# WangXuan95/NBLIC-Image-Compression

Hardware: AMD Instinct MI355X
Metric: Mpixel/s encode (bit-exact) 4096x4096 gray -e1 lossless (higher is better)
Workload: dtype u8

## Files before the change

include/nblic_amd.h:

```cpp
#ifndef NBLIC_AMD_H
#define NBLIC_AMD_H

#include <stddef.h>
#include <stdint.h>

#ifdef __cplusplus
extern "C" {
#endif

#define NBLIC_MAX_HEIGHT     65535
#define NBLIC_MAX_WIDTH      65535
#define NBLIC_MAX_IMG_SIZE   100000000
#define QNBLIC_MAX_HEIGHT    65535
#define QNBLIC_MAX_WIDTH     65535
#define QNBLIC_MAX_IMG_SIZE  100000000


int NBLICcompress(int verbose, unsigned char *p_buf, unsigned char *p_img, int height, int width,
                  int *p_near, int *p_effort);

int NBLICdecompress(int verbose, unsigned char *p_buf, unsigned char *p_img, int *p_height, int *p_width,
                    int *p_near, int *p_effort);

int QNBLICcompress(uint16_t *p_buf, unsigned char *p_img, int height, int width);
// ... 5 lines not shown

nblic_amd_ctx *nblic_amd_create(int device, int n_slots, int n_coders);

nblic_amd_ctx *nblic_amd_create_ex(int device, int n_groups, int group_size, int n_coders, int n_host_buffers);
void nblic_amd_destroy(nblic_amd_ctx *ctx);

int nblic_amd_encode_batch(nblic_amd_ctx *ctx, int n_images, const unsigned char *const *imgs, int imgs_on_device,
                           const int *heights, const int *widths, unsigned char *const *outs,
                           const size_t *out_caps, long *out_lens);

typedef struct nblic_amd_batch nblic_amd_batch;
nblic_amd_batch *nblic_amd_encode_batch_begin(nblic_amd_ctx *ctx, int n_images, const unsigned char *const *imgs,
                                              int imgs_on_device, const int *heights, const int *widths,
                                              unsigned char *const *outs, const size_t *out_caps, long *out_lens);
int nblic_amd_encode_batch_end(nblic_amd_ctx *ctx, nblic_amd_batch *batch);

int nblic_amd_qencode_batch(nblic_amd_ctx *ctx, int n_images, const unsigned char *const *imgs, int imgs_on_device,
                            const int *heights, const int *widths, uint16_t *const *outs, const size_t *out_caps_words,
                            long *out_len_words);

int nblic_amd_encode_batch_modes(nblic_amd_ctx *ctx, int n_images, const unsigned char *const *imgs, int imgs_on_device,
                                 const int *heights, const int *widths, const int *nears, const int *efforts,
                                 unsigned char *const *outs, const size_t *out_caps, long *out_lens,
                                 unsigned char *const *recons);

int nblic_amd_decode_batch(nblic_amd_ctx *ctx, int n_images, const unsigned char *const *streams, const size_t *stream_lens,
                           unsigned char *const *imgs, const size_t *img_caps, int *heights, int *widths, int *nears,
                           int *efforts, int *status);

int nblic_amd_set_device_coder(nblic_amd_ctx *ctx, int n_packs, int min_outstanding);
void nblic_amd_device_coder_stats(nblic_amd_ctx *ctx, double *bins, long *packs, long *images);

int nblic_amd_copy_stats(nblic_amd_ctx *ctx, long out[4]);

void nblic_amd_set_max_pixels(nblic_amd_ctx *ctx, long max_pixels);

void nblic_amd_set_serial_rows(nblic_amd_ctx *ctx, int rows);
long nblic_amd_serial_launches(nblic_amd_ctx *ctx);

void nblic_amd_set_long_chains(nblic_amd_ctx *ctx, int min_records, int block_records);
int nblic_amd_long_chain_stats(nblic_amd_ctx *ctx, long counts[8], int reset);

int nblic_amd_lsq_redo_counts(nblic_amd_ctx *ctx, unsigned long long counts[2], int reset);

int nblic_amd_serial_plan(int decode, int effort, int images, int width, int whole_streams);

typedef struct nblic_amd_stream nblic_amd_stream;
nblic_amd_stream *nblic_amd_stream_begin(nblic_amd_ctx *ctx, const unsigned char *img, int img_on_device, int height, int width,
                                         int near, int effort, int band_rows);
nblic_amd_stream *nblic_amd_stream_resume(nblic_amd_ctx *ctx, const unsigned char *img, int img_on_device, const void *checkpoint,
                                          size_t checkpoint_bytes);
int nblic_amd_stream_run(nblic_amd_stream *s, double budget_seconds, unsigned char *out, size_t out_cap, size_t *out_len);
size_t nblic_amd_stream_checkpoint(nblic_amd_stream *s, void *buf, size_t cap);
int nblic_amd_stream_check(nblic_amd_ctx *ctx, const void *checkpoint, size_t bytes);
int nblic_amd_stream_progress(nblic_amd_stream *s, int *rows_done, unsigned long long *bytes_total, unsigned char sha256[32], double *model_ms);
int nblic_amd_stream_recon(nblic_amd_stream *s, unsigned char *plane, int *first_row, int *end_row);
void nblic_amd_stream_end(nblic_amd_stream *s);
int nblic_amd_stream_set_index(nblic_amd_stream *s, int every_rows);
size_t nblic_amd_stream_index(nblic_amd_stream *s, void *buf, size_t cap);
int nblic_amd_stream_set_front(nblic_amd_stream *s, int front);

typedef struct nblic_amd_dstream nblic_amd_dstream;
nblic_amd_dstream *nblic_amd_dstream_begin(nblic_amd_ctx *ctx, int band_rows);
nblic_amd_dstream *nblic_amd_dstream_resume(nblic_amd_ctx *ctx, const void *checkpoint, size_t bytes);
int nblic_amd_dstream_check(nblic_amd_ctx *ctx, const void *checkpoint, size_t bytes);
int nblic_amd_dstream_feed(nblic_amd_dstream *d, const unsigned char *bytes, size_t n, int final_);
// ... 375 lines not shown
```

nblic-image-compression_amd/__init__.py:

```python
from __future__ import annotations

import ctypes as C
import os
import subprocess
import weakref
from typing import List, Optional, Sequence, Tuple

import numpy as np


_HERE = os.path.dirname(os.path.abspath(__file__))
LIB_PATH = os.environ.get("NBLIC_AMD_LIB") or os.path.join(_HERE, "libnblic_amd.so")
CSRC = os.path.join(_HERE, "csrc")
INCLUDE = os.path.join(os.path.dirname(_HERE), "include", "nblic_amd.h")

_u8p = C.POINTER(C.c_uint8)
_lib = None

EXPORTS = (
    "NBLICcompress", "NBLICdecompress", "QNBLICcompress", "QNBLICdecompress", "QNBLICcompressMultiThread",
    "nblic_amd_create", "nblic_amd_create_ex", "nblic_amd_destroy", "nblic_amd_encode_batch", "nblic_amd_encode_batch_begin", "nblic_amd_encode_batch_end", "nblic_amd_qencode_batch", "nblic_amd_set_max_pixels",
    "nblic_amd_enable_timing", "nblic_amd_stage_times", "nblic_amd_last_launches", "nblic_amd_last_stats", "nblic_amd_debug_stage", "nblic_amd_debug_live", "nblic_amd_debug_takes", "nblic_amd_debug_pack_rows", "nblic_amd_debug_device_code", "nblic_amd_debug_model_stages", "nblic_amd_debug_back_half", "nblic_amd_debug_entropy_front",
    "nblic_amd_encode_batch_modes", "nblic_amd_decode_batch", "nblic_amd_serial_selftest",
    "nblic_amd_set_serial_rows", "nblic_amd_serial_launches", "nblic_amd_set_long_chains", "nblic_amd_long_chain_stats", "nblic_amd_lsq_redo_counts", "nblic_amd_serial_plan", "nblic_amd_lsq_probe", "nblic_amd_set_feed_chunk", "nblic_amd_last_fed_bytes",
    "nblic_amd_stream_begin", "nblic_amd_stream_resume", "nblic_amd_stream_run", "nblic_amd_stream_checkpoint", "nblic_amd_stream_progress",
    "nblic_amd_stream_recon", "nblic_amd_stream_end", "nblic_amd_stream_check",
    "nblic_amd_dstream_begin", "nblic_amd_dstream_resume", "nblic_amd_dstream_check", "nblic_amd_dstream_feed", "nblic_amd_dstream_info",
    "nblic_amd_dstream_run", "nblic_amd_dstream_progress", "nblic_amd_dstream_checkpoint", "nblic_amd_dstream_end",
    "nblic_amd_index_check", "nblic_amd_index_build", "nblic_amd_decode_indexed", "nblic_amd_decode_rows",
    "nblic_amd_stream_set_index", "nblic_amd_stream_index", "nblic_amd_set_index_round", "nblic_amd_stream_set_front",
    "nblic_amd_encode_batch_indexed", "nblic_amd_index_bytes", "nblic_amd_indexed_batch_split",
    "nblic_amd_qencode_batch_indexed", "nblic_amd_debug_q_entropy",
    "nblic_amd_set_device_qcoder", "nblic_amd_device_qcoder_stats", "nblic_amd_qcoder_selftest", "nblic_amd_debug_q_rans_host", "nblic_amd_debug_device_q_entropy",
    "nblic_amd_decode_batch_indexed", "nblic_amd_indexed_decode_split", "nblic_amd_indexed_decode_plan", "nblic_amd_debug_index_kernels",
    "nblic_amd_index_build_batch", "nblic_amd_index_build_split", "nblic_amd_index_build_plan", "nblic_amd_debug_index_capture",
    "nblic_amd_index_pack", "nblic_amd_index_pack_bound", "nblic_amd_index_unpack", "nblic_amd_index_unpacked_bytes", "nblic_amd_index_is_packed", "nblic_amd_debug_index_unpack",
    "nblic_amd_decode_batch_indexed_to", "nblic_amd_decode_batch_to", "nblic_amd_debug_deliver_host", "nblic_amd_debug_deliver",
    "nblic_amd_decode_batch_indexed_to_ex", "nblic_amd_decode_batch_to_ex", "nblic_amd_deliver_stats", "nblic_amd_debug_deliver_host_ex", "nblic_amd_debug_deliver_ex",
    "nblic_amd_encode_batch_modes_from_to",
    "nblic_amd_encode_batch_modes_from", "nblic_amd_qencode_batch_from", "nblic_amd_encode_batch_indexed_from", "nblic_amd_qencode_batch_indexed_from",
    "nblic_amd_collect_stats", "nblic_amd_collect_ms", "nblic_amd_debug_collect_host", "nblic_amd_debug_collect",
    "nblic_amd_debug_collect_ref_host", "nblic_amd_debug_collect_ref", "nblic_amd_debug_deliver_ref_host", "nblic_amd_debug_deliver_ref",
    "nblic_amd_color_plan", "nblic_amd_color_choose", "nblic_amd_color_mode_valid", "nblic_amd_color_mode_ref", "nblic_amd_color_plan_stats",
    "nblic_amd_encode_batch_modes_from_color", "nblic_amd_qencode_batch_from_color", "nblic_amd_encode_batch_indexed_from_color",
    "nblic_amd_qencode_batch_indexed_from_color", "nblic_amd_decode_batch_to_ex_color", "nblic_amd_decode_batch_indexed_to_ex_color",
    "nblic_amd_debug_color_cost_host", "nblic_amd_debug_color_cost",
    "nblic_amd_stack_plan", "nblic_amd_stack_choose", "nblic_amd_stack_slice_mode", "nblic_amd_stack_mode_valid", "nblic_amd_stack_modes_valid", "nblic_amd_stack_plan_stats",
    "nblic_amd_encode_batch_modes_from_stack", "nblic_amd_qencode_batch_from_stack", "nblic_amd_encode_batch_indexed_from_stack",
    "nblic_amd_qencode_batch_indexed_from_stack", "nblic_amd_decode_batch_to_ex_stack", "nblic_amd_decode_batch_indexed_to_ex_stack",
    "nblic_amd_debug_stack_deliver_host", "nblic_amd_debug_stack_deliver", "nblic_amd_debug_stack_cost_host", "nblic_amd_debug_stack_cost",
    "nblic_amd_deep_plan", "nblic_amd_deep_choose", "nblic_amd_deep_mode_valid", "nblic_amd_deep_plan_stats",
    "nblic_amd_encode_batch_modes_from_deep", "nblic_amd_qencode_batch_from_deep", "nblic_amd_encode_batch_indexed_from_deep",
    "nblic_amd_qencode_batch_indexed_from_deep", "nblic_amd_decode_batch_to_ex_deep", "nblic_amd_decode_batch_indexed_to_ex_deep",
    "nblic_amd_debug_deep_collect_host", "nblic_amd_debug_deep_collect", "nblic_amd_debug_deep_deliver_host", "nblic_amd_debug_deep_deliver",
    "nblic_amd_debug_deep_cost_host", "nblic_amd_debug_deep_cost",
    "nblic_amd_cli_main", "nblic_amd_cli_parse", "nblic_amd_read_gray", "nblic_amd_write_gray",
    "nblic_amd_set_device_coder", "nblic_amd_device_coder_stats", "nblic_amd_copy_stats",
    "nblic_amd_range_code", "nblic_amd_range_code_multi", "nblic_amd_range_code_chunked", "nblic_amd_range_code_packs", "nblic_amd_pack_groups_host", "nblic_amd_selftest", "nblic_amd_syn1", "nblic_amd_version",
)


def build(force: bool = False) -> str:
    srcs = [os.path.join(CSRC, f) for f in os.listdir(CSRC)] + [INCLUDE]
    stale = force or not os.path.exists(LIB_PATH) or any(os.path.getmtime(s) > os.path.getmtime(LIB_PATH) for s in srcs)
    if stale:
        r = subprocess.run(["make", "-C", CSRC], capture_output=True, text=True)
        if r.returncode != 0:
            raise RuntimeError("building libnblic_amd.so failed:\n" + r.stdout + r.stderr)
    return LIB_PATH


def load_library() -> C.CDLL:
    global _lib
    if _lib is not None:
        return _lib
    if not os.path.exists(LIB_PATH):
        raise RuntimeError(f"{LIB_PATH} is missing: run __graft_entry__.build() (hipcc, gfx950). "
                           "There is no CPU fallback for the NBLIC hot path.")
    lib = C.CDLL(LIB_PATH)
    ip = C.POINTER(C.c_int)
    lib.NBLICcompress.restype = C.c_int
    lib.NBLICcompress.argtypes = [C.c_int, _u8p, _u8p, C.c_int, C.c_int, ip, ip]
    lib.NBLICdecompress.restype = C.c_int
    lib.NBLICdecompress.argtypes = [C.c_int, _u8p, _u8p, ip, ip, ip, ip]
    u16p = C.POINTER(C.c_uint16)
    lib.QNBLICcompress.restype = C.c_int
    lib.QNBLICcompress.argtypes = [u16p, _u8p, C.c_int, C.c_int]
    lib.QNBLICcompressMultiThread.restype = C.c_int
    lib.QNBLICcompressMultiThread.argtypes = [u16p, _u8p, C.c_int, C.c_int]
    lib.QNBLICdecompress.restype = C.c_int
# ... 19 lines not shown
    lib.nblic_amd_encode_batch_modes.argtypes = [C.c_void_p, C.c_int, C.POINTER(C.c_void_p), C.c_int, ip, ip, ip, ip,
                                                 C.POINTER(C.c_void_p), C.POINTER(C.c_size_t), C.POINTER(C.c_long), C.POINTER(C.c_void_p)]
    lib.nblic_amd_decode_batch.restype = C.c_int
    lib.nblic_amd_decode_batch.argtypes = [C.c_void_p, C.c_int, C.POINTER(C.c_void_p), C.POINTER(C.c_size_t), C.POINTER(C.c_void_p),
                                           C.POINTER(C.c_size_t), ip, ip, ip, ip, ip]
    lib.nblic_amd_serial_selftest.restype = C.c_int
    lib.nblic_amd_serial_selftest.argtypes = [C.c_void_p]
    lib.nblic_amd_cli_main.restype = C.c_int
    lib.nblic_amd_cli_main.argtypes = [C.c_int, C.POINTER(C.c_char_p)]
    lib.nblic_amd_cli_parse.restype = None
    lib.nblic_amd_cli_parse.argtypes = [C.c_int, C.POINTER(C.c_char_p), ip, C.c_char_p, C.c_char_p, C.c_size_t]
    lib.nblic_amd_read_gray.restype = C.c_int
    lib.nblic_amd_read_gray.argtypes = [C.c_char_p, _u8p, C.c_size_t, ip, ip]
    lib.nblic_amd_write_gray.restype = C.c_int
    lib.nblic_amd_write_gray.argtypes = [C.c_char_p, _u8p, C.c_int, C.c_int, C.c_int]
    lib.nblic_amd_set_device_coder.restype = C.c_int
    lib.nblic_amd_set_device_coder.argtypes = [C.c_void_p, C.c_int, C.c_int]
    lib.nblic_amd_device_coder_stats.restype = None
    lib.nblic_amd_device_coder_stats.argtypes = [C.c_void_p, C.POINTER(C.c_double), C.POINTER(C.c_long), C.POINTER(C.c_long)]
    lib.nblic_amd_set_max_pixels.restype = None
    lib.nblic_amd_set_max_pixels.argtypes = [C.c_void_p, C.c_long]
    lib.nblic_amd_set_serial_rows.restype = None
    lib.nblic_amd_set_serial_rows.argtypes = [C.c_void_p, C.c_int]
    lib.nblic_amd_serial_launches.restype = C.c_long
    lib.nblic_amd_serial_launches.argtypes = [C.c_void_p]
    if hasattr(lib, "nblic_amd_set_long_chains"):
        lib.nblic_amd_set_long_chains.restype = None
        lib.nblic_amd_set_long_chains.argtypes = [C.c_void_p, C.c_int, C.c_int]
        lib.nblic_amd_long_chain_stats.restype = C.c_int
        lib.nblic_amd_long_chain_stats.argtypes = [C.c_void_p, C.POINTER(C.c_long), C.c_int]
    if hasattr(lib, "nblic_amd_copy_stats"):
        lib.nblic_amd_copy_stats.restype = C.c_int
        lib.nblic_amd_copy_stats.argtypes = [C.c_void_p, C.POINTER(C.c_long)]
    lib.nblic_amd_lsq_redo_counts.restype = C.c_int
    lib.nblic_amd_lsq_redo_counts.argtypes = [C.c_void_p, C.POINTER(C.c_ulonglong), C.c_int]
    lib.nblic_amd_serial_plan.restype = C.c_int
    lib.nblic_amd_serial_plan.argtypes = [C.c_int, C.c_int, C.c_int, C.c_int, C.c_int]
    lib.nblic_amd_lsq_probe.restype = C.c_int
    lib.nblic_amd_lsq_probe.argtypes = [C.c_void_p, C.c_int, C.c_int, C.c_int, C.POINTER(C.c_double), C.POINTER(C.c_int8), ip,
                                        C.POINTER(C.c_double), C.POINTER(C.c_longlong)]
    lib.nblic_amd_set_feed_chunk.restype = None
    lib.nblic_amd_set_feed_chunk.argtypes = [C.c_void_p, C.c_size_t]
    lib.nblic_amd_last_fed_bytes.restype = C.c_long
    lib.nblic_amd_last_fed_bytes.argtypes = [C.c_void_p]
    lib.nblic_amd_stream_begin.restype = C.c_void_p
    lib.nblic_amd_stream_begin.argtypes = [C.c_void_p, C.c_void_p, C.c_int, C.c_int, C.c_int, C.c_int, C.c_int, C.c_int]
    lib.nblic_amd_stream_resume.restype = C.c_void_p
    lib.nblic_amd_stream_resume.argtypes = [C.c_void_p, C.c_void_p, C.c_int, C.c_void_p, C.c_size_t]
    lib.nblic_amd_stream_run.restype = C.c_int
    lib.nblic_amd_stream_run.argtypes = [C.c_void_p, C.c_double, C.c_void_p, C.c_size_t, C.POINTER(C.c_size_t)]
    lib.nblic_amd_stream_checkpoint.restype = C.c_size_t
    lib.nblic_amd_stream_checkpoint.argtypes = [C.c_void_p, C.c_void_p, C.c_size_t]
    lib.nblic_amd_stream_progress.restype = C.c_int
    lib.nblic_amd_stream_progress.argtypes = [C.c_void_p, ip, C.POINTER(C.c_ulonglong), C.c_void_p, C.POINTER(C.c_double)]
    lib.nblic_amd_stream_recon.restype = C.c_int
    lib.nblic_amd_stream_recon.argtypes = [C.c_void_p, C.c_void_p, ip, ip]
    lib.nblic_amd_stream_end.restype = None
    lib.nblic_amd_stream_end.argtypes = [C.c_void_p]
    lib.nblic_amd_stream_check.restype = C.c_int
    lib.nblic_amd_stream_check.argtypes = [C.c_void_p, C.c_void_p, C.c_size_t]
    lib.nblic_amd_dstream_begin.restype = C.c_void_p
    lib.nblic_amd_dstream_begin.argtypes = [C.c_void_p, C.c_int]
    lib.nblic_amd_dstream_resume.restype = C.c_void_p
    lib.nblic_amd_dstream_resume.argtypes = [C.c_void_p, C.c_void_p, C.c_size_t]
    lib.nblic_amd_dstream_check.restype = C.c_int
    lib.nblic_amd_dstream_check.argtypes = [C.c_void_p, C.c_void_p, C.c_size_t]
# ... 2374 lines not shown
            raise RuntimeError("nblic_amd_debug_index_unpack failed (%d)" % rc)
        res = []
        for out, stride, (_, _, walk, first_out) in zip(outs, strides, tasks):
            used = (int(walk) - int(first_out)) * int(stride)
            res.append((out[:used].reshape(-1, int(stride)), out[used:used + 256]))
        return res

    def set_index_round(self, segments: int):
        self.lib.nblic_amd_set_index_round(self.handle, int(segments))

    def set_serial_rows(self, rows: int):
        self.lib.nblic_amd_set_serial_rows(self.handle, rows)

    def serial_launches(self) -> int:
        return int(self.lib.nblic_amd_serial_launches(self.handle))

    LONG_CHAIN_COUNTS = ("s2_met", "s2_table", "s2_serial", "s3_split", "s3_accepted", "s3_missed")

    def set_long_chains(self, min_records: int = 0, block_records: int = 0):
        self.lib.nblic_amd_set_long_chains(self.handle, min_records, block_records)

    def long_chain_stats(self, reset: bool = False) -> dict:
        v = (C.c_long * 8)()
        if self.lib.nblic_amd_long_chain_stats(self.handle, v, int(reset)) != 0:
            raise RuntimeError("nblic_amd_long_chain_stats failed")
        return dict(zip(self.LONG_CHAIN_COUNTS, (int(x) for x in v)))

    def copy_stats(self) -> dict:
        v = (C.c_long * 4)()
        if self.lib.nblic_amd_copy_stats(self.handle, v) != 0:
            raise RuntimeError("nblic_amd_copy_stats failed")
        return {"engine": int(v[0]), "runtime": int(v[1]), "fallbacks": int(v[2]), "available": bool(v[3])}

    def lsq_redo_counts(self, reset: bool = False) -> Tuple[int, int]:
        return _lsq_redo_counts(self.handle, reset)

    def lsq_probe(self, n: int, waves: int, stats: np.ndarray, regressors: np.ndarray, bias: np.ndarray):
        stats = np.ascontiguousarray(stats, np.float64)
        regressors = np.ascontiguousarray(regressors, np.int8)
        bias = np.ascontiguousarray(bias, np.int32)
        k = int(bias.shape[0])
        assert stats.shape == (k, 1 + n + n * n) and regressors.shape == (k, 10)
        of, oi = np.zeros((k, 12), np.float64), np.zeros((k, 14), np.int64)
        rc = self.lib.nblic_amd_lsq_probe(self.handle, n, waves, k, stats.ctypes.data_as(C.POINTER(C.c_double)),
                                          regressors.ctypes.data_as(C.POINTER(C.c_int8)), bias.ctypes.data_as(C.POINTER(C.c_int)),
                                          of.ctypes.data_as(C.POINTER(C.c_double)), oi.ctypes.data_as(C.POINTER(C.c_longlong)))
        if rc != 0:
            raise RuntimeError("nblic_amd_lsq_probe failed")
        return of, oi

    def encode_ptrs(self, ptrs: Sequence[int], shapes: Sequence[Tuple[int, int]], on_device: bool,
                    outs: Optional[List[np.ndarray]] = None) -> Tuple[List[np.ndarray], np.ndarray]:
        k = len(ptrs)
        if outs is None:
            outs = [np.empty(out_capacity(h, w), np.uint8) for (h, w) in shapes]
        imgs, hs, ws, op, caps, lens = _batch_args(ptrs, shapes, outs)
        rc = self.lib.nblic_amd_encode_batch(self.handle, k, imgs, int(on_device), hs, ws, op, caps, lens)
        arr = np.array(list(lens), dtype=np.int64)
        if rc != 0:
            raise RuntimeError(f"nblic_amd_encode_batch failed (lengths {arr.tolist()})")
        return outs, arr

    def encode_begin(self, ptrs: Sequence[int], shapes: Sequence[Tuple[int, int]], on_device: bool,
                     outs: Optional[List[np.ndarray]] = None):
        k = len(ptrs)
        if outs is None:
# ... 546 lines not shown
```

nblic-image-compression_amd/csrc/pipeline.hip:

```cpp
#include <hip/hip_runtime.h>

#include <algorithm>
#include <atomic>
#include <chrono>
#include <condition_variable>
#include <cstdio>
#include <cstdlib>
#include <cstring>
#include <deque>
#include <functional>
#include <memory>
#include <mutex>
#include <thread>
#include <type_traits>
#include <vector>

#include <pthread.h>
#include <sched.h>
#include <fcntl.h>
#include <unistd.h>

#include "../../include/nblic_amd.h"
#include "device_coder.h"
#include "hip_owned.h"
#include "index_entries.h"
#include "index_pack.h"
#include "kernels_e1.h"
#include "lsq_f64.h"
#include "model.h"
#include "q_device_coder.h"
#include "q_entropy.h"
#include "range_coder.h"
#include "serial_engine.h"
#include "sha256.h"

struct nblic_amd_ctx;

namespace nblic {

#define HIP_OK(call)                                                                          \
    do {                                                                                      \
        hipError_t e_ = (call);                                                               \
        if (e_ != hipSuccess) {                                                               \
            fprintf(stderr, "[nblic_amd] %s failed: %s (%s:%d)\n", #call, hipGetErrorString(e_), __FILE__, __LINE__); \
            return false;                                                                     \
        }                                                                                     \
    } while (0)

enum DbgFlag : int {
    kDbgDeviceOnly = 16,
    kDbgReport = 32,
    kDbgTrace = 64,
    kDbgFeedOnly = 128,
    kDbgNoCopy = 1024,
};
static int dbg_flags() {
    static const int flags = [] { const char *v = getenv("NBLIC_AMD_DBG"); return v ? atoi(v) : 0; }();
    return flags;
}

void RangeScalar::feed(const uint16_t *coded, size_t n) {
    if (overflow) return;
    uint32_t l = lo, h = hi;
    uint8_t *q = p;
// ... 174 lines not shown
    double dev_bins = 0; long dev_packs = 0, dev_images = 0;
    std::thread qdev;
    int qmode = 0;
    uint32_t q_budget = 0;
    double qdev_symbols = 0, qdev_kernel_ms = 0; long qdev_launches = 0, qdev_images = 0;
    Stream dec_stream, dec_stream2;
    DevBuf<uint8_t> dec_arena;
    DevBuf<SerialJob> dec_jobs;
    int index_round_segments = 0;
    int serial_rows = 0;
    DevBuf<unsigned long long> d_redo;
    double idx_split[5] = {0}; long idx_steps = 0;
    double idxbuild_split[4] = {0};
    double idxdec_split[4] = {0};
    int long_min = 0, long_block = 0;
    long long_counts[8] = {0};
    long serial_launch_count = 0;
    size_t feed_chunk = size_t(1) << 20;
    long fed_bytes = 0;
    int feed_pipe[2] = {-1, -1};
    DevBuf<DeliverTask> dec_deliver;
    DevBuf<StackDeliverTask> dec_runs;
    DevBuf<StackSlice> dec_slices;
    std::atomic<long> collect_counts[4] = {};
    double collect_ms = 0; long collect_timed = 0;
    std::atomic<long> color_counts[2] = {};
    double color_ms = 0;
    std::atomic<long> stack_counts[4] = {};
    double stack_ms = 0, stack_deliver_ms = 0;
    long deliver_tasks = 0, deliver_strided = 0;
    DevBuf<DeepDeliverTask> dec_deep;
    std::atomic<long> deep_counts[4] = {};
    double deep_ms[3] = {0, 0, 0};
};

namespace nblic {

static int take_group(nblic_amd_ctx *c) {
    std::unique_lock<std::mutex> l(c->fm);
    c->fcv.wait(l, [c] { return !c->free_groups.empty(); });
    const int id = c->free_groups.front();
    c->free_groups.pop_front();
    return id;
}

static void release_group(nblic_amd_ctx *c, int id) {
    { std::lock_guard<std::mutex> g(c->fm); c->free_groups.push_back(id); }
    c->fcv.notify_all();
}

static bool nothing_outstanding(nblic_amd_ctx *c) {
    std::lock_guard<std::mutex> l(c->fm);
    return c->coding == 0;
}

static void return_coded(nblic_amd_ctx *c, Slot &s) {
    if (s.cb < 0) return;
    {
        std::lock_guard<std::mutex> l(c->fm);
        if (s.pack_n <= 1) c->free_cbufs.push_front(s.cb);
        else if (s.pack_lane == 0) c->free_pbufs.push_front(s.cb);
    }
    s.cb = -1; s.pack_n = 1; s.pack_lane = 0;
    c->fcv.notify_all();
}

static void finish_images(nblic_amd_ctx *c, const ReadyImage *im, int n) {
    {
        std::lock_guard<std::mutex> l(c->fm);
        for (int k = 0; k < n; k++) {
            if (im[k].pack_n <= 1) c->free_cbufs.push_front(im[k].cb);
            else if (im[k].pack_lane == 0) c->free_pbufs.push_front(im[k].cb);
            im[k].batch->remaining -= 1;
        }
        c->coding -= n;
    }
    c->fcv.notify_all();
}

static uint8_t *begin_stream_out(const ReadyImage &im, size_t *room) {
    const size_t cap = std::min(im.caps[im.job], size_t(1) << 46);
    *room = cap >= size_t(kHeaderBytes) ? cap - kHeaderBytes : 0;
    if (cap >= size_t(kHeaderBytes)) write_header(im.outs[im.job], im.h, im.w, im.near, im.k_step, im.effort);
    return im.outs[im.job] + kHeaderBytes;
}

static bool group_init(Group &g, int id, int n_slots, nblic_amd_ctx *c) {
    g.id = id; g.ctx = c;
    g.slots.resize(size_t(n_slots));
    HIP_OK(g.stream.create(hipStreamNonBlocking));
    HIP_OK(g.done.create(hipEventDisableTiming | hipEventBlockingSync));
    if (c->engine.available()) HIP_OK(g.released.create(hipEventDisableTiming | hipEventReleaseToSystem));
    for (int k = 0; k < kE1Marks; k++) { HIP_OK(g.tm_ev[k].create(hipEventDefault)); g.tm.ev[k] = g.tm_ev[k]; }
    HIP_OK(g.h_jobs.alloc(size_t(n_slots))); HIP_OK(g.d_jobs.alloc(size_t(n_slots)));
    HIP_OK(g.h_sjobs.alloc(size_t(n_slots))); HIP_OK(g.d_sjobs.alloc(size_t(n_slots)));
    HIP_OK(g.h_totals.alloc(size_t(n_slots) * kTotalsSlot)); HIP_OK(g.d_totals.alloc(size_t(n_slots) * kTotalsSlot));
    for (int k = 0; k < n_slots; k++) {
        Slot &s = g.slots[size_t(k)];
        DevPool &m = s.mem;
        HIP_OK(m.renew(s.b.table, size_t(4096) * kMaxSegments)); HIP_OK(m.renew(s.b.scan_sums, (size_t(1) << 20) / sizeof(uint32_t)));
        s.b.totals = g.d_totals + size_t(k) * kTotalsSlot;
        HIP_OK(m.renew(s.b.ctx_state, 4096));
        HIP_OK(m.renew(s.b.qhist, 12 * 256)); HIP_OK(m.renew(s.b.map_state, 512 * 60)); HIP_OK(m.renew(s.b.cnt_state, 4096 * 2));
        HIP_OK(m.renew(s.b.win_base, 4097 + 4096)); HIP_OK(m.renew(s.b.blk_base, 4097)); HIP_OK(m.renew(s.b.mblk_base, 513)); HIP_OK(m.renew(s.b.mend_cnt, 512 * 20)); HIP_OK(m.renew(s.b.dbg_out, 4096));
        HIP_OK(hipMemset(s.b.dbg_out, 0, 4096 * sizeof(unsigned long long)));
        uint8_t *state = nullptr;
        HIP_OK(m.renew(state, kModelStateBytes));
        s.d_state = reinterpret_cast<SerialState *>(state);
    }
    return true;
}

static bool ensure_events(Slot &s, size_t n_ev) {
    if (n_ev <= s.ev_cap) return true;
    const size_t cap = n_ev + n_ev / 8 + 1024;
    DevPool &m = s.mem;
    s.ev_cap = 0;
    HIP_OK(m.renew(s.b.events, cap)); HIP_OK(m.renew(s.b.tin, 2 * cap + kStreamPad)); HIP_OK(m.renew(s.b.tpos, cap + 64));
    HIP_OK(m.renew(s.b.tout, 2 * cap + kStreamPad)); HIP_OK(m.renew(s.b.win_recs, (2 * cap / 512 + 4096 + 8) * 24));
    s.ev_cap = cap;
    return true;
}

// ... 3779 lines not shown
        for (int j = 0; j < w; j++) {
            xs ^= xs << 13; xs ^= xs >> 17; xs ^= xs << 5;
            int t = ((i + 2 * j) >> 3) & 511;
            int base = iabs(t - 256); if (base > 255) base = 255;
            int v = ((base * 3) >> 2) + 32 + ((i ^ j) & 15) + int(xs & 7) + int((xs >> 3) & 7) - 7;
            img[size_t(i) * size_t(w) + size_t(j)] = uint8_t(iclip(v, 0, 255));
        }
}

const char *nblic_amd_version(void) { return "nblic_amd 0.2 (NBLIC v0.3 bitstream, gfx950)"; }

nblic_amd_ctx *nblic_amd_create_ex(int device, int n_groups, int group_size, int n_coders, int n_host_buffers) {
    int count = 0;
    if (hipGetDeviceCount(&count) != hipSuccess || count <= 0) {
        fprintf(stderr, "[nblic_amd] no HIP device available -- this library has no CPU fallback\n");
        return nullptr;
    }
    if (device < 0 || device >= count || hipSetDevice(device) != hipSuccess) {
        fprintf(stderr, "[nblic_amd] cannot select HIP device %d of %d\n", device, count);
        return nullptr;
    }
    if (n_groups < 1) n_groups = 1;
    if (group_size < 1) group_size = 1;
    if (n_coders < 1) n_coders = 1;
    if (n_host_buffers < n_groups * group_size + kMaxTake) n_host_buffers = n_groups * group_size + kMaxTake;
    auto *c = new nblic_amd_ctx;
    c->device = device;
    c->simd = have_avx512() && !getenv("NBLIC_AMD_NO_SIMD");
    {
        const char *ce = getenv("NBLIC_AMD_COPY_ENGINE");
        if (!ce || atoi(ce) != 0) c->engine.open();
    }
    c->groups.resize(size_t(n_groups));
    for (int i = 0; i < n_groups; i++) {
        if (!group_init(c->groups[size_t(i)], i, group_size, c)) { nblic_amd_destroy(c); return nullptr; }
        c->free_groups.push_back(i);
    }
    c->cbufs.resize(size_t(n_host_buffers));
    for (int i = 0; i < n_host_buffers; i++) c->free_cbufs.push_back(i);
    const int n_pack_buffers = std::max(n_groups * ((group_size + int(kPackLanes) - 1) / int(kPackLanes)) + kMaxPacks, n_host_buffers / int(kPackLanes));
    c->pbufs.resize(size_t(n_pack_buffers));
    for (int i = 0; i < n_pack_buffers; i++) c->free_pbufs.push_back(i);
    if (c->dec_stream.create(hipStreamNonBlocking) != hipSuccess || c->d_redo.alloc(2) != hipSuccess || hipMemset(c->d_redo, 0, 2 * sizeof(unsigned long long)) != hipSuccess ||
        c->dec_stream2.create(hipStreamNonBlocking) != hipSuccess) { nblic_amd_destroy(c); return nullptr; }
    if (const char *cb = getenv("NBLIC_AMD_CHUNK_BINS")) {
        const size_t v = size_t(atol(cb));
        if (v >= 4096 && v <= kChunkBins) c->chunk_bins = v & ~(kGroupBins - 1);
    }
    int n_copy = n_coders < kCopyStreams ? n_coders : kCopyStreams;
    if (const char *cs = getenv("NBLIC_AMD_COPY_STREAMS")) { const int v = atoi(cs); if (v >= 1 && v <= 32) n_copy = v; }
    c->copy_streams.resize(size_t(n_copy));
    for (auto &cs : c->copy_streams)
        if (cs.create(hipStreamNonBlocking) != hipSuccess) { nblic_amd_destroy(c); return nullptr; }
    c->coders_wanted = n_coders;
    if (const char *mt = getenv("NBLIC_AMD_MAX_TAKE")) { const int v = atoi(mt); if (v >= 2 && v <= kMaxTake) c->max_take = v; }
    for (int i = 0; i < n_coders; i++) c->coders.emplace_back(coder_main, c, i);
    for (int i = 0; i < n_groups; i++) c->drivers.emplace_back(driver_main, c, i);
    c->submitter = std::thread(submitter_main, c);
    return c;
}

nblic_amd_ctx *nblic_amd_create(int device, int n_slots, int n_coders) {
    if (n_slots < 1) n_slots = 1;
    int n_groups = n_slots >= 2 ? 2 : 1;
    return nblic_amd_create_ex(device, n_groups, (n_slots + n_groups - 1) / n_groups, n_coders, 2 * n_slots);
}

void nblic_amd_destroy(nblic_amd_ctx *c) {
// ... 1228 lines not shown
            if (gate_status[s] != -1) S[s].gate = d_gates + s;
        }
        if (!stack_task_ok(runs[i], S.data())) return -1;
    }
    std::vector<uint8_t> back(std::max<size_t>(outs_total, 1));
    std::vector<SerialState> gates(total);
    for (size_t s = 0; s < total; s++) gates[s].status = gate_status[s];
    const bool ok = [&]() -> bool {
        HIP_OK(hipMemsetAsync(d_planes, 0, planes_total, st));
        HIP_OK(hipMemsetAsync(d_outs, kPattern, std::max<size_t>(outs_total, 256), st));
        HIP_OK(hipMemcpyAsync(d_gates, gates.data(), total * sizeof(SerialState), hipMemcpyHostToDevice, st));
        for (size_t s = 0; s < total; s++) HIP_OK(hipMemcpyAsync(d_planes + plane_at[s] + base_offsets[s], planes[s], plane_len[s], hipMemcpyHostToDevice, st));
        c->stack_counts[2] += 1; c->stack_counts[3] += long(count);
        unsigned long long chunks = 0;
        if (!deliver_stack_upload(runs.data(), count, S.data(), total, d_runs, d_slices, st, chunks) || !deliver_stack_launch(d_runs, n, d_slices, uint32_t(chunks), st)) return false;
        if (outs_total) HIP_OK(hipMemcpyAsync(back.data(), d_outs, outs_total, hipMemcpyDeviceToHost, st));
        HIP_OK(hipStreamSynchronize(st));
        return true;
    }();
    if (st) hipStreamSynchronize(st);
    if (!ok) return -2;
    for (size_t s = 0; s < total; s++) if (outs[s]) memcpy(outs[s], back.data() + out_at[s], out_bytes[s]);
    return 0;
}

void nblic_amd_debug_live(long counts[4]) { for (int k = 0; k < 4; k++) counts[k] = g_live[k].load(std::memory_order_relaxed); }

int nblic_amd_copy_stats(nblic_amd_ctx *c, long out[4]) {
    if (!c || !out) return -1;
    c->engine.stats(out);
    return 0;
}

void nblic_amd_set_max_pixels(nblic_amd_ctx *c, long max_pixels) {
    if (!c) c = default_ctx();
    if (c) c->max_px = max_pixels > 0 ? max_pixels : kMaxPixels;
}
void nblic_amd_set_serial_rows(nblic_amd_ctx *c, int rows) {
    if (!c) c = default_ctx();
    if (c) { std::lock_guard<std::mutex> g(c->api); c->serial_rows = rows > 0 ? rows : 0; }
}
void nblic_amd_set_long_chains(nblic_amd_ctx *c, int min_records, int block_records) {
    if (!c) c = default_ctx();
    if (c) { std::lock_guard<std::mutex> g(c->api); c->long_min = min_records < 0 ? -1 : min_records; c->long_block = block_records > 0 ? block_records : 0; }
}
int nblic_amd_long_chain_stats(nblic_amd_ctx *c, long counts[8], int reset) {
    if (!c) c = default_ctx();
    if (!c || !counts) return -1;
    std::lock_guard<std::mutex> l(c->stat_m);
    for (int k = 0; k < 8; k++) { counts[k] = c->long_counts[k]; if (reset) c->long_counts[k] = 0; }
    return 0;
}
long nblic_amd_serial_launches(nblic_amd_ctx *c) {
    if (!c) c = default_ctx();
    if (!c) return -1;
    std::lock_guard<std::mutex> l(c->stat_m);
    return c->serial_launch_count;
}
int nblic_amd_lsq_redo_counts(nblic_amd_ctx *c, unsigned long long counts[2], int reset) {
    if (!c) c = default_ctx();
    if (!c || !counts) return -1;
    std::lock_guard<std::mutex> g(c->api);
    unsigned long long v[2] = {0, 0};
    if (hipSetDevice(c->device) != hipSuccess || hipMemcpy(v, c->d_redo, sizeof v, hipMemcpyDeviceToHost) != hipSuccess) return -1;
    if (reset && hipMemset(c->d_redo, 0, sizeof v) != hipSuccess) return -1;
    counts[0] = v[0]; counts[1] = v[1];
// ... 1173 lines not shown
```

Measured before the change: 5310.

## Probe HIP streams for shared hardware queues and spread groups evenly across them

At context creation, the code creates candidate non-blocking streams and probes which ones share a hardware queue. It does this by timing whether an empty kernel on one stream waits behind a busy kernel on another. It then picks one stream per group so the groups are balanced across the distinct queue classes, and drops the extra candidates. The aim is to stop several encode groups from serializing on the same hardware queue when the runtime deals streams out unevenly. The cost is a one-time probing step, which can be switched off with NBLIC_AMD_QUEUE_PLAN=0, and the plan depends on timing heuristics that may come back inconclusive.

```diff
diff --git a/include/nblic_amd.h b/include/nblic_amd.h
--- a/include/nblic_amd.h
+++ b/include/nblic_amd.h
@@ -61,6 +61,8 @@
 void nblic_amd_device_coder_stats(nblic_amd_ctx *ctx, double *bins, long *packs, long *images);
 
 int nblic_amd_copy_stats(nblic_amd_ctx *ctx, long out[4]);
+
+int nblic_amd_queue_plan_stats(nblic_amd_ctx *ctx, long out[40], double *plan_ms);
 
 void nblic_amd_set_max_pixels(nblic_amd_ctx *ctx, long max_pixels);
 
diff --git a/nblic-image-compression_amd/__init__.py b/nblic-image-compression_amd/__init__.py
--- a/nblic-image-compression_amd/__init__.py
+++ b/nblic-image-compression_amd/__init__.py
@@ -55,7 +55,7 @@
     "nblic_amd_debug_deep_collect_host", "nblic_amd_debug_deep_collect", "nblic_amd_debug_deep_deliver_host", "nblic_amd_debug_deep_deliver",
     "nblic_amd_debug_deep_cost_host", "nblic_amd_debug_deep_cost",
     "nblic_amd_cli_main", "nblic_amd_cli_parse", "nblic_amd_read_gray", "nblic_amd_write_gray",
-    "nblic_amd_set_device_coder", "nblic_amd_device_coder_stats", "nblic_amd_copy_stats",
+    "nblic_amd_set_device_coder", "nblic_amd_device_coder_stats", "nblic_amd_copy_stats", "nblic_amd_queue_plan_stats",
     "nblic_amd_range_code", "nblic_amd_range_code_multi", "nblic_amd_range_code_chunked", "nblic_amd_range_code_packs", "nblic_amd_pack_groups_host", "nblic_amd_selftest", "nblic_amd_syn1", "nblic_amd_version",
 )
 
@@ -141,6 +141,9 @@
     if hasattr(lib, "nblic_amd_copy_stats"):
         lib.nblic_amd_copy_stats.restype = C.c_int
         lib.nblic_amd_copy_stats.argtypes = [C.c_void_p, C.POINTER(C.c_long)]
+    if hasattr(lib, "nblic_amd_queue_plan_stats"):
+        lib.nblic_amd_queue_plan_stats.restype = C.c_int
+        lib.nblic_amd_queue_plan_stats.argtypes = [C.c_void_p, C.POINTER(C.c_long), C.POINTER(C.c_double)]
     lib.nblic_amd_lsq_redo_counts.restype = C.c_int
     lib.nblic_amd_lsq_redo_counts.argtypes = [C.c_void_p, C.POINTER(C.c_ulonglong), C.c_int]
     lib.nblic_amd_serial_plan.restype = C.c_int
@@ -2581,6 +2584,15 @@
             raise RuntimeError("nblic_amd_copy_stats failed")
         return {"engine": int(v[0]), "runtime": int(v[1]), "fallbacks": int(v[2]), "available": bool(v[3])}
 
+    QUEUE_PLAN_STATES = ("on", "few_groups", "switched_off", "one_class", "inconclusive", "error")
+
+    def queue_plan(self) -> dict:
+        v, ms = (C.c_long * 40)(), C.c_double(0.0)
+        if self.lib.nblic_amd_queue_plan_stats(self.handle, v, C.byref(ms)) != 0:
+            raise RuntimeError("nblic_amd_queue_plan_stats failed")
+        return {"state": self.QUEUE_PLAN_STATES[int(v[0])], "on": int(v[0]) == 0, "classes": int(v[1]), "candidates": int(v[2]), "n_groups": int(v[3]),
+                "spread": int(v[4]), "unplanned_spread": int(v[5]), "groups_per_class": [int(v[8 + k]) for k in range(int(v[1]))], "plan_ms": float(ms.value)}
+
     def lsq_redo_counts(self, reset: bool = False) -> Tuple[int, int]:
         return _lsq_redo_counts(self.handle, reset)
 
diff --git a/nblic-image-compression_amd/csrc/pipeline.hip b/nblic-image-compression_amd/csrc/pipeline.hip
--- a/nblic-image-compression_amd/csrc/pipeline.hip
+++ b/nblic-image-compression_amd/csrc/pipeline.hip
@@ -30,6 +30,7 @@
 #include "model.h"
 #include "q_device_coder.h"
 #include "q_entropy.h"
+#include "queue_plan.h"
 #include "range_coder.h"
 #include "serial_engine.h"
 #include "sha256.h"
@@ -270,6 +271,7 @@
     DevBuf<DeepDeliverTask> dec_deep;
     std::atomic<long> deep_counts[4] = {};
     double deep_ms[3] = {0, 0, 0};
+    QueuePlan queue_plan;
 };
 
 namespace nblic {
@@ -323,10 +325,89 @@
     return im.outs[im.job] + kHeaderBytes;
 }
 
-static bool group_init(Group &g, int id, int n_slots, nblic_amd_ctx *c) {
+__global__ void k_queue_probe_busy(unsigned long long ticks, unsigned cap) {
+    const unsigned long long t0 = __builtin_amdgcn_s_memtime();
+    for (unsigned i = 0; i < cap; i++) {
+        if (__builtin_amdgcn_s_memtime() - t0 >= ticks) break;
+        __builtin_amdgcn_s_sleep(16);
+    }
+}
+__global__ void k_queue_probe_empty() {}
+
+struct QueueProbe {
+    static constexpr unsigned kCap = 20000;
+    static constexpr double kWantMs = 1.0;
+    unsigned long long ticks = 2000000;
+    double busy_ms = 0;
+    static double ms_since(std::chrono::steady_clock::time_point t0) { return std::chrono::duration<double, std::milli>(std::chrono::steady_clock::now() - t0).count(); }
+    int measure(hipStream_t a) {
+        busy_ms = 1e30;
+        for (int rep = 0; rep < 3; rep++) {
+            const auto t0 = std::chrono::steady_clock::now();
+            hipLaunchKernelGGL(k_queue_probe_busy, dim3(1), dim3(64), 0, a, ticks, kCap);
+            if (hipGetLastError() != hipSuccess || hipStreamSynchronize(a) != hipSuccess) return kProbeError;
+            busy_ms = std::min(busy_ms, ms_since(t0));
+        }
+        return kProbeFree;
+    }
+    int calibrate(hipStream_t a) {
+        hipLaunchKernelGGL(k_queue_probe_empty, dim3(1), dim3(64), 0, a);
+        if (hipGetLastError() != hipSuccess || hipStreamSynchronize(a) != hipSuccess) return kProbeError;
+        int r = measure(a);
+        if (r != kProbeFree) return r;
+        if (busy_ms < 0.5 * kWantMs && busy_ms > 0.001) {
+            ticks = (unsigned long long)(double(ticks) * kWantMs / busy_ms);
+            if ((r = measure(a)) != kProbeFree) return r;
+        }
+        return busy_ms >= 0.3 * kWantMs && busy_ms <= 20.0 * kWantMs ? kProbeFree : kProbeInconclusive;
+    }
+    int blocks(hipStream_t a, hipStream_t b) {
+        for (int rep = 0; rep < 3; rep++) {
+            hipLaunchKernelGGL(k_queue_probe_busy, dim3(1), dim3(64), 0, a, ticks, kCap);
+            if (hipGetLastError() != hipSuccess) return kProbeError;
+            const auto t0 = std::chrono::steady_clock::now();
+            hipLaunchKernelGGL(k_queue_probe_empty, dim3(1), dim3(64), 0, b);
+            const bool ok = hipGetLastError() == hipSuccess && hipStreamSynchronize(b) == hipSuccess;
+            const double ms = ms_since(t0);
+            if (hipStreamSynchronize(a) != hipSuccess || !ok) return kProbeError;
+            if (ms < 0.5 * busy_ms) return kProbeFree;
+        }
+        return kProbeBlocks;
+    }
+};
+
+static void plan_group_streams(nblic_amd_ctx *c, int n_groups, std::vector<Stream> &streams) {
+    QueuePlan &p = c->queue_plan;
+    p.n_groups = n_groups;
+    if (n_groups < 3) { p.state = kPlanFewGroups; return; }
+    if (const char *v = getenv("NBLIC_AMD_QUEUE_PLAN")) if (atoi(v) == 0) { p.state = kPlanSwitchedOff; }
+    if (p.state != kPlanSwitchedOff) {
+        const auto t0 = std::chrono::steady_clock::now();
+        std::vector<Stream> cand;
+        QueueProbe probe;
+        bool calibrated = false;
+        p = plan_queues(n_groups,
+            [&]() -> int {
+                cand.emplace_back();
+                if (cand.back().create(hipStreamNonBlocking) != hipSuccess) { cand.pop_back(); return -1; }
+                return int(cand.size()) - 1;
+            },
+            [&](int a, int b) -> int {
+                if (!calibrated) { const int r = probe.calibrate(cand[size_t(a)]); if (r != kProbeFree) return r; calibrated = true; }
+                return probe.blocks(cand[size_t(a)], cand[size_t(b)]);
+            },
+            [&](int id) { cand[size_t(id)] = Stream(); });
+        if (p.state == kPlanOn) for (int id : p.chosen) streams.push_back(std::move(cand[size_t(id)]));
+        p.plan_ms = QueueProbe::ms_since(t0);
+    }
+    if (p.state != kPlanOn) fprintf(stderr, "[nblic_amd] queue plan off (%s): one stream per group as the runtime deals them\n", queue_plan_state_name(p.state));
+}
+
+static bool group_init(Group &g, int id, int n_slots, nblic_amd_ctx *c, Stream *planned = nullptr) {
     g.id = id; g.ctx = c;
     g.slots.resize(size_t(n_slots));
-    HIP_OK(g.stream.create(hipStreamNonBlocking));
+    if (planned) g.stream = std::move(*planned);
+    else HIP_OK(g.stream.create(hipStreamNonBlocking));
     HIP_OK(g.done.create(hipEventDisableTiming | hipEventBlockingSync));
     if (c->engine.available()) HIP_OK(g.released.create(hipEventDisableTiming | hipEventReleaseToSystem));
     for (int k = 0; k < kE1Marks; k++) { HIP_OK(g.tm_ev[k].create(hipEventDefault)); g.tm.ev[k] = g.tm_ev[k]; }
@@ -4172,8 +4253,10 @@
         if (!ce || atoi(ce) != 0) c->engine.open();
     }
     c->groups.resize(size_t(n_groups));
+    std::vector<Stream> planned;
+    plan_group_streams(c, n_groups, planned);
     for (int i = 0; i < n_groups; i++) {
-        if (!group_init(c->groups[size_t(i)], i, group_size, c)) { nblic_amd_destroy(c); return nullptr; }
+        if (!group_init(c->groups[size_t(i)], i, group_size, c, planned.empty() ? nullptr : &planned[size_t(i)])) { nblic_amd_destroy(c); return nullptr; }
         c->free_groups.push_back(i);
     }
     c->cbufs.resize(size_t(n_host_buffers));
@@ -5468,6 +5551,17 @@
     return 0;
 }
 
+int nblic_amd_queue_plan_stats(nblic_amd_ctx *c, long out[40], double *plan_ms) {
+    static_assert(kPlanMaxClasses == 32, "the header says 8 + 32 values");
+    if (!c || !out) return -1;
+    const QueuePlan &p = c->queue_plan;
+    std::fill(out, out + 40, 0L);
+    out[0] = p.state; out[1] = p.classes; out[2] = p.candidates; out[3] = p.n_groups; out[4] = p.spread(); out[5] = p.unplanned_spread();
+    for (int k = 0; k < p.classes; k++) out[8 + k] = p.groups_per_class[k];
+    if (plan_ms) *plan_ms = p.plan_ms;
+    return 0;
+}
+
 void nblic_amd_set_max_pixels(nblic_amd_ctx *c, long max_pixels) {
     if (!c) c = default_ctx();
     if (c) c->max_px = max_pixels > 0 ? max_pixels : kMaxPixels;
diff --git a/nblic-image-compression_amd/csrc/queue_plan.h b/nblic-image-compression_amd/csrc/queue_plan.h
--- /dev/null
+++ b/nblic-image-compression_amd/csrc/queue_plan.h
@@ -0,0 +1,112 @@
+#pragma once
+#include <algorithm>
+#include <vector>
+
+namespace nblic {
+
+constexpr int kPlanMaxClasses = 32;
+
+enum QueuePlanState {
+    kPlanOn = 0,
+    kPlanFewGroups = 1,
+    kPlanSwitchedOff = 2,
+    kPlanOneClass = 3,
+    kPlanInconclusive = 4,
+    kPlanError = 5,
+};
+inline const char *queue_plan_state_name(int s) {
+    static const char *const names[] = {"on", "fewer than three groups", "switched off (NBLIC_AMD_QUEUE_PLAN=0)", "one class found", "a probe was inconclusive", "a runtime call failed"};
+    return s >= 0 && s < 6 ? names[s] : "?";
+}
+
+enum ProbeAnswer { kProbeFree = 0, kProbeBlocks = 1, kProbeInconclusive = -1, kProbeError = -2 };
+
+struct QueuePlan {
+    int state = kPlanFewGroups;
+    int n_groups = 0;
+    int classes = 0;
+    int candidates = 0;
+    int groups_per_class[kPlanMaxClasses] = {0};
+    int unplanned_per_class[kPlanMaxClasses] = {0};
+    double plan_ms = 0;
+    std::vector<int> chosen;
+    std::vector<int> chosen_class;
+    static int spread_of(const int *v, int n) { return n > 0 ? *std::max_element(v, v + n) - *std::min_element(v, v + n) : 0; }
+    int spread() const { return spread_of(groups_per_class, classes); }
+    int unplanned_spread() const { return spread_of(unplanned_per_class, classes); }
+    int most() const { return classes > 0 ? *std::max_element(groups_per_class, groups_per_class + classes) : 0; }
+    int unplanned_most() const { return classes > 0 ? *std::max_element(unplanned_per_class, unplanned_per_class + classes) : 0; }
+};
+
+namespace plan_detail {
+inline bool split(int n, const std::vector<int> &members, std::vector<int> &share) {
+    share.assign(members.size(), 0);
+    for (int g = 0; g < n; g++) {
+        int best = -1;
+        for (size_t k = 0; k < members.size(); k++)
+            if (share[k] < members[k] && (best < 0 || share[k] < share[size_t(best)])) best = int(k);
+        if (best < 0) return false;
+        share[size_t(best)]++;
+    }
+    return true;
+}
+}
+
+template <class NewCandidate, class Blocks, class Drop>
+inline QueuePlan plan_queues(int n_groups, NewCandidate new_candidate, Blocks blocks, Drop drop) {
+    QueuePlan p;
+    p.n_groups = n_groups;
+    if (n_groups < 3) { p.state = kPlanFewGroups; return p; }
+    std::vector<std::vector<int>> cls;
+    std::vector<int> all, members, share;
+    auto give_up = [&](int state) {
+        for (int id : all) drop(id);
+        p.state = state; p.classes = int(cls.size()); p.chosen.clear(); p.chosen_class.clear();
+        std::fill(p.groups_per_class, p.groups_per_class + kPlanMaxClasses, 0);
+        std::fill(p.unplanned_per_class, p.unplanned_per_class + kPlanMaxClasses, 0);
+        if (state != kPlanOneClass) p.classes = 0;
+        else p.groups_per_class[0] = p.unplanned_per_class[0] = n_groups;
+        return p;
+    };
+    const int cap = 4 * n_groups;
+    while (p.candidates < cap) {
+        const int id = new_candidate();
+        if (id < 0) return give_up(kPlanError);
+        all.push_back(id); p.candidates++;
+        int k = 0;
+        for (; k < int(cls.size()); k++) {
+            const int a = blocks(cls[size_t(k)][0], id);
+            if (a == kProbeError) return give_up(kPlanError);
+            if (a == kProbeInconclusive) return give_up(kPlanInconclusive);
+            if (a == kProbeBlocks) break;
+        }
+        if (k == int(cls.size())) {
+            if (k == kPlanMaxClasses) return give_up(kPlanInconclusive);
+            cls.emplace_back();
+        }
+        cls[size_t(k)].push_back(id);
+        if (p.candidates <= n_groups) p.unplanned_per_class[k]++;
+        if (p.candidates < n_groups) continue;
+        if (int(cls.size()) >= n_groups) break;
+        if (p.candidates >= 2 * n_groups) {
+            members.clear();
+            for (auto &c : cls) members.push_back(int(c.size()));
+            if (plan_detail::split(n_groups, members, share) && QueuePlan::spread_of(share.data(), int(share.size())) <= 1) break;
+        }
+    }
+    if (cls.size() <= 1) return give_up(kPlanOneClass);
+    members.clear();
+    for (auto &c : cls) members.push_back(int(c.size()));
+    plan_detail::split(n_groups, members, share);
+    p.classes = int(cls.size());
+    std::vector<char> kept(size_t(*std::max_element(all.begin(), all.end())) + 1, 0);
+    for (size_t k = 0; k < cls.size(); k++) {
+        p.groups_per_class[k] = share[k];
+        for (int j = 0; j < share[k]; j++) { p.chosen.push_back(cls[k][size_t(j)]); p.chosen_class.push_back(int(k)); kept[size_t(cls[k][size_t(j)])] = 1; }
+    }
+    for (int id : all) if (!kept[size_t(id)]) drop(id);
+    p.state = kPlanOn;
+    return p;
+}
+
+}
```

After: 5841, median of 6. +10.0%, better.
